# dhmodi/spark-timeseries

Hardware: AMD Instinct MI355X
Metric: series fitted/sec, ARIMA(2,1,2) CSS-CGD, 1M x 1024 pts (higher is better)
Workload: dtype f64; 1 GPU; ARIMA(2,1,2)+c css-cgd, 1048576 series x 1024 pts per GPU (BASELINE.json configs[1]/[2]); series_per_gpu=1048576, series_total=1048576, series_len=1024, parallelism=series-sharded x1, no collective, breeze_overlap=smear, fit_kernel=k_cg_fit (LDS slots, 1 wave/SIMD), fit_pipeline=6, hw_queues=8, series_done=1048576

## Files before the change

spark-timeseries_amd/csrc/arima_device.hpp:

```cpp
#pragma once

#include <hip/hip_runtime.h>
#include <stdint.h>

#include <type_traits>

#include "../../include/sparkts_arima.h"
#include "arima_launch.hpp"
#include "cg_lane.hpp"

namespace sts {

constexpr int kChunk = 16;


__device__ __forceinline__ double dlog(double x) {
    const double ln2_hi = 6.93147180369123816490e-01, ln2_lo = 1.90821492927058770002e-10,
                 two54 = 1.80143985094819840000e+16, Lg1 = 6.666666666666735130e-01,
                 Lg2 = 3.999999999940941908e-01, Lg3 = 2.857142874366239149e-01,
                 Lg4 = 2.222219843214978396e-01, Lg5 = 1.818357216161805012e-01,
                 Lg6 = 1.531383769920937332e-01, Lg7 = 1.479819860511658591e-01;
    int64_t bits = __double_as_longlong(x);
    int32_t hx = (int32_t)(bits >> 32);
    uint32_t lx = (uint32_t)bits;
    int32_t k = 0;
    if (hx < 0x00100000) {
        if (((hx & 0x7fffffff) | lx) == 0) return -two54 / 0.0;
        if (hx < 0) return (x - x) / 0.0;
        k -= 54;
        x *= two54;
        hx = (int32_t)(__double_as_longlong(x) >> 32);
    }
    if (hx >= 0x7ff00000) return x + x;
    k += (hx >> 20) - 1023;
    hx &= 0x000fffff;
    int32_t i = (hx + 0x95f64) & 0x100000;
    {
        uint64_t u = (uint64_t)__double_as_longlong(x);
        u = ((uint64_t)(uint32_t)(hx | (i ^ 0x3ff00000)) << 32) | (u & 0xffffffffull);
        x = __longlong_as_double((long long)u);
    }
    k += (i >> 20);
    double f = x - 1.0;
    double dk;
    if ((0x000fffff & (2 + hx)) < 3) {
        if (f == 0.0) {
            if (k == 0) return 0.0;
            dk = (double)k;
            return dk * ln2_hi + dk * ln2_lo;
        }
        double R = f * f * (0.5 - 0.33333333333333333 * f);
        if (k == 0) return f - R;
        dk = (double)k;
        return dk * ln2_hi - ((R - dk * ln2_lo) - f);
    }
    double s = f / (2.0 + f);
    dk = (double)k;
    double z = s * s;
    i = hx - 0x6147a;
    double w = z * z;
    int32_t j = 0x6b851 - hx;
    double t1 = w * (Lg2 + w * (Lg4 + w * Lg6));
    double t2 = z * (Lg1 + w * (Lg3 + w * (Lg5 + w * Lg7)));
    i |= j;
    double R = t2 + t1;
    if (i > 0) {
        double hfsq = 0.5 * f * f;
        if (k == 0) return f - (hfsq - s * (hfsq + R));
        return dk * ln2_hi - ((hfsq - (s * (hfsq + R) + dk * ln2_lo)) - f);
    }
    if (k == 0) return f - s * (f - R);
    return dk * ln2_hi - ((s * (f - R) - dk * ln2_lo) - f);
}

__device__ __forceinline__ double css_to_loglik(double css, int n) {
    double sigma2 = css / (double)n;
    return (double)(-n / 2) * dlog(2.0 * 3.141592653589793 * sigma2) - css / (2.0 * sigma2);
}

struct Chunk {
    double v[kChunk];
};

__device__ __forceinline__ void load_chunk(const double *__restrict__ p, Chunk &out) {
    const double2 *q = reinterpret_cast<const double2 *>(p);
#pragma unroll
    for (int u = 0; u < kChunk / 2; ++u) {
        const double2 t = q[u];
        out.v[2 * u] = t.x;
        out.v[2 * u + 1] = t.y;
    }
}

template <int D, class Fn>
__device__ __forceinline__ void stream_elems(const double *__restrict__ row, int first, int last, Fn &&fn) {
    if (first >= last) return;
    const int c_first = first / kChunk;
    const int c_last = (last - 1) / kChunk;
    const int nch = c_last - c_first + 1;
    const double *base = row + c_first * kChunk;
    Chunk ring[D];
#pragma unroll
    for (int j = 0; j < D; ++j) load_chunk(base + (j < nch ? j : nch - 1) * kChunk, ring[j]);
    const int head = first - c_first * kChunk;
    const int tail = last - c_last * kChunk;
    for (int c0 = 0; c0 < nch; c0 += D) {
#pragma unroll
        for (int j = 0; j < D; ++j) {
            const int ch = c0 + j;
            if (ch < nch) {
                const bool full = (ch > 0 || head == 0) && (ch < nch - 1 || tail == kChunk);
                if (full) {
#pragma unroll
                    for (int u = 0; u < kChunk; ++u) fn(ring[j].v[u]);
                } else {
                    const int lo = (ch == 0) ? head : 0;
                    const int hi = (ch == nch - 1) ? tail : kChunk;
#pragma unroll
                    for (int u = 0; u < kChunk; ++u)
                        if (u >= lo && u < hi) fn(ring[j].v[u]);
                }
            }
            const int nx = ch + D;
            load_chunk(base + (nx < nch ? nx : nch - 1) * kChunk, ring[j]);
        }
    }
}

__device__ __forceinline__ double drow_at(const double *__restrict__ raw, int dd, int i) {
    return dd ? raw[i + 1] - raw[i] : raw[i];
}

template <int D, class Fn>
__device__ __forceinline__ void stream_row(const double *__restrict__ raw, int dd, int first, int last, Fn &&fn) {
    if (first >= last) return;
    const int off = (int)((reinterpret_cast<uintptr_t>(raw) >> 3) & (kChunk - 1));
    double prev = raw[first];
    stream_elems<D>(raw - off, first + dd + off, last + dd + off, [&](double x) {
        const double v = dd ? x - prev : x;
        prev = x;
        fn(v);
    });
}

constexpr int kPrefetchF = 3;
constexpr int kPrefetchG = 1;

template <int P, int Q, int I, bool G, bool SMEAR, bool RAW = false, int DPF = (G ? kPrefetchG : kPrefetchF)>
__device__ __forceinline__ void css_pass(const double *__restrict__ row, int n,
                                         const double (&c)[I + P + Q > 0 ? I + P + Q : 1], double &css_out,
                                         double (&g)[I + P + Q > 0 ? I + P + Q : 1], int dd = 0) {
    constexpr int K = I + P + Q;
    constexpr int KA = K > 0 ? K : 1;
    constexpr int M = (P > Q ? P : Q);
    constexpr int PA = P > 0 ? P : 1;
    double yl[PA];
#pragma unroll
    for (int j = 0; j < PA; ++j) {
        if constexpr (RAW) yl[j] = (j < P && M - 1 - j < n) ? drow_at(row, dd, M - 1 - j) : 0.0;
        else yl[j] = (j < P) ? row[M - 1 - j] : 0.0;
    }
    double e1 = 0.0, e2 = 0.0, css = 0.0, sigma2 = 0.0;
    const double yh0 = 0.0 + (double)I * c[0];
    const double nd = (double)n;
    constexpr int DER = G ? (SMEAR ? (Q > 0 ? 2 : 1) : Q + 1) : 1;
    double dE[DER][KA];
    if constexpr (G) {
#pragma unroll
        for (int r = 0; r < DER; ++r)
#pragma unroll
            for (int j = 0; j < KA; ++j) dE[r][j] = 0.0;
    }
#pragma unroll
    for (int j = 0; j < KA; ++j) g[j] = 0.0;

    auto step = [&](double yi) {
        if constexpr (!G) {
            double yh = yh0;
#pragma unroll
            for (int j = 0; j < P; ++j) yh = yh + yl[j] * c[I + j];
#pragma unroll
            for (int j = 0; j < Q; ++j) yh = yh + (j == 0 ? e1 : e2) * c[I + P + j];
            const double e = yi - yh;
            css = css + e * e;
            e2 = e1;
            e1 = e;
        } else {
#pragma unroll
            for (int j = 0; j < K; ++j)
#pragma unroll
                for (int kk = 0; kk < Q; ++kk) dE[0][j] = dE[0][j] - c[I + P + kk] * dE[SMEAR ? DER - 1 : kk + 1][j];
            double yh = yh0;
            if constexpr (K > 0) dE[0][0] = dE[0][0] - (double)I;
#pragma unroll
            for (int j = 0; j < P; ++j) {
                yh = yh + yl[j] * c[I + j];
                dE[0][I + j] = dE[0][I + j] - yl[j];
            }
#pragma unroll
            for (int j = 0; j < Q; ++j) {
                const double mj = (j == 0 ? e1 : e2);
                yh = yh + mj * c[I + P + j];
                dE[0][I + P + j] = dE[0][I + P + j] - mj;
            }
            const double e = yi - yh;
            const double e_sq = e * e;
            sigma2 = sigma2 + e_sq / nd;
            css = css + e_sq;
            e2 = e1;
            e1 = e;
#pragma unroll
            for (int j = 0; j < K; ++j) g[j] = g[j] + dE[0][j] * e;
            if constexpr (SMEAR) {
                if constexpr (Q > 0) {
#pragma unroll
                    for (int j = 0; j < KA; ++j) dE[1][j] = dE[0][j];
                }
            } else {
#pragma unroll
                for (int r = Q; r >= 1; --r)
#pragma unroll
                    for (int j = 0; j < KA; ++j) dE[r][j] = dE[r - 1][j];
            }
#pragma unroll
            for (int j = 0; j < KA; ++j) dE[0][j] = 0.0;
        }
        if constexpr (P > 0) {
#pragma unroll
            for (int j = PA - 1; j >= 1; --j) yl[j] = yl[j - 1];
            yl[0] = yi;
        }
    };
    if constexpr (RAW) stream_row<DPF>(row, dd, M, n, step);
    else stream_elems<DPF>(row, M, n, step);
    css_out = css;
    if constexpr (G) {
#pragma unroll
        for (int j = 0; j < KA; ++j) g[j] = g[j] / -sigma2;
    }
}

template <int P, int Q, int I, int NCH, int DPF = kPrefetchF>
__device__ __forceinline__ void css_pass_multi(const double *__restrict__ row, int n,
                                               const double (&c)[NCH][I + P + Q > 0 ? I + P + Q : 1],
                                               double (&css_out)[NCH], int dd = 0) {
    constexpr int M = (P > Q ? P : Q);
    constexpr int PA = P > 0 ? P : 1;
    double yl[PA];
#pragma unroll
    for (int j = 0; j < PA; ++j) yl[j] = (j < P && M - 1 - j < n) ? drow_at(row, dd, M - 1 - j) : 0.0;
    double e1[NCH], e2[NCH], css[NCH], yh0[NCH];
#pragma unroll
    for (int h = 0; h < NCH; ++h) {
        e1[h] = e2[h] = css[h] = 0.0;
        yh0[h] = 0.0 + (double)I * c[h][0];
    }
    auto step = [&](double yi) {
#pragma unroll
        for (int h = 0; h < NCH; ++h) {
            double yh = yh0[h];
#pragma unroll
            for (int j = 0; j < P; ++j) yh = yh + yl[j] * c[h][I + j];
#pragma unroll
            for (int j = 0; j < Q; ++j) yh = yh + (j == 0 ? e1[h] : e2[h]) * c[h][I + P + j];
            const double e = yi - yh;
            css[h] = css[h] + e * e;
            e2[h] = e1[h];
            e1[h] = e;
        }
        if constexpr (P > 0) {
#pragma unroll
            for (int j = PA - 1; j >= 1; --j) yl[j] = yl[j - 1];
            yl[0] = yi;
        }
    };
    stream_row<DPF>(row, dd, M, n, step);
#pragma unroll
    for (int h = 0; h < NCH; ++h) css_out[h] = css[h];
}

template <int P, int Q, int I>
__device__ __forceinline__ double css_row_lds(const double *row, int n,
                                              const double (&c)[I + P + Q > 0 ? I + P + Q : 1]) {
    constexpr int M = (P > Q ? P : Q);
    constexpr int PA = P > 0 ? P : 1;
    double yl[PA];
#pragma unroll
    for (int j = 0; j < PA; ++j) yl[j] = (j < P && M - 1 - j >= 0 && M - 1 - j < n) ? row[M - 1 - j] : 0.0;
    double e1 = 0.0, e2 = 0.0, css = 0.0;
    const double yh0 = 0.0 + (double)I * c[0];
// ... 264 lines not shown
    constexpr int DR = SMEAR ? 1 : (Q > 0 ? Q : 1);
    double yl[PA];
#pragma unroll
    for (int j = 0; j < PA; ++j) yl[j] = (j < P && M - 1 - j >= 0 && M - 1 - j < n) ? row[M - 1 - j] : 0.0;
    double e1 = 0.0, e2 = 0.0, css = 0.0, sigma2 = 0.0, g = 0.0;
    double dl[DR];
#pragma unroll
    for (int r = 0; r < DR; ++r) dl[r] = 0.0;
    const double yh0 = 0.0 + (double)I * c[0];
    const double nd = (double)n;
#pragma unroll 4
    for (int t = M; t < n; ++t) {
        const double yi = row[t];
        double d0 = 0.0;
#pragma unroll
        for (int kk = 0; kk < Q; ++kk) d0 = d0 - c[I + P + kk] * dl[SMEAR ? 0 : kk];
        double dv = 0.0;
        if constexpr (I) dv = (col == 0) ? 1.0 : dv;
        double yh = yh0;
#pragma unroll
        for (int j = 0; j < P; ++j) {
            yh = yh + yl[j] * c[I + j];
            dv = (col == I + j) ? yl[j] : dv;
        }
#pragma unroll
        for (int j = 0; j < Q; ++j) {
            const double mj = (j == 0 ? e1 : e2);
            yh = yh + mj * c[I + P + j];
            dv = (col == I + P + j) ? mj : dv;
        }
        d0 = d0 - dv;
        const double e = yi - yh;
        const double e_sq = e * e;
        sigma2 = sigma2 + e_sq / nd;
        css = css + e_sq;
        e2 = e1;
        e1 = e;
        g = g + d0 * e;
        if constexpr (Q > 0) {
            if constexpr (SMEAR) {
                dl[0] = d0;
            } else {
#pragma unroll
                for (int r = DR - 1; r >= 1; --r) dl[r] = dl[r - 1];
                dl[0] = d0;
            }
        }
        if constexpr (P > 0) {
#pragma unroll
            for (int j = PA - 1; j >= 1; --j) yl[j] = yl[j - 1];
            yl[0] = yi;
        }
    }
    css_out = css;
    g_out = g / -sigma2;
}

constexpr int kPrefetchHR = 2;

template <int C>
struct HouseholderState {
    double a[C];
    double vtop[C];
    double alpha[C][C];
    double dot[C];
};

template <int C>
__device__ __forceinline__ void hh_apply(const HouseholderState<C> &H, int s, double (&x)[C], double &y) {
#pragma unroll
    for (int j = 0; j < C; ++j) {
        if (j < s) {
            const double v = x[j];
#pragma unroll
            for (int c = j + 1; c < C; ++c) x[c] = x[c] - H.alpha[j][c] * v;
            y = y + H.dot[j] * v;
        }
    }
}

template <class Gen, class Fn>
__device__ __forceinline__ void gen_stream(const Gen &gen, const double *__restrict__ row, int first, int last,
                                           Fn &&fn) {
    if constexpr (Gen::kFuse) stream_row<kPrefetchHR>(row, gen.dd, first, last, fn);
    else stream_row<kPrefetchHR>(row, 0, first, last, fn);
}

template <int C, int S, class Gen>
__device__ __forceinline__ int ols_stage(Gen &gen, const double *__restrict__ row, int n, int R,
                                         HouseholderState<C> &H) {
    if constexpr (S == C) {
        return ARIMA_ST_OK;
    } else {
        double xs[C], ys;
        gen.row_at(S, xs, ys);
        hh_apply<C>(H, S, xs, ys);
        const double xss = xs[S];
        double xnorm = 0.0 + xss * xss;
        if constexpr (S == 0 && Gen::kOnesFirst) {
            xnorm = (double)R;
        } else if (S + 1 < R) {
            gen.begin(S + 1);
            gen_stream(gen, row, gen.first_elem(S + 1), n, [&](double v) {
                double x[C], y;
                gen.push(v, x, y);
                hh_apply<C>(H, S, x, y);
                xnorm = xnorm + x[S] * x[S];
            });
        }
        const double a = (xss > 0) ? -sqrt(xnorm) : sqrt(xnorm);
        H.a[S] = a;
        if (a == 0.0) return ARIMA_ST_SINGULAR;
        const double vt = xss - a;
        H.vtop[S] = vt;
        double al[C], dt;
#pragma unroll
        for (int c = 0; c < C; ++c) al[c] = (c > S) ? 0.0 - xs[c] * vt : 0.0;
        dt = 0.0 + ys * vt;
        if (S + 1 < R) {
            gen.begin(S + 1);
            gen_stream(gen, row, gen.first_elem(S + 1), n, [&](double v) {
                double x[C], y;
                gen.push(v, x, y);
                hh_apply<C>(H, S, x, y);
                const double vs = x[S];
#pragma unroll
                for (int c = S + 1; c < C; ++c) al[c] = al[c] - x[c] * vs;
                dt = dt + y * vs;
            });
        }
        const double den = a * vt;
#pragma unroll
        for (int c = 0; c < C; ++c) H.alpha[S][c] = (c > S) ? al[c] / den : 0.0;
        H.dot[S] = dt / den;
        return ols_stage<C, S + 1>(gen, row, n, R, H);
    }
}

template <int C, class Gen>
__device__ __forceinline__ int stream_ols(Gen &gen, const double *__restrict__ row, int n, int R, double (&beta)[C]) {
    HouseholderState<C> H;
    const int st = ols_stage<C, 0>(gen, row, n, R, H);
    if (st != ARIMA_ST_OK) return st;
    double rrow[C][C];
    double ytop[C];
#pragma unroll
    for (int i = 0; i < C; ++i) {
        double x[C], y;
        gen.row_at(i, x, y);
        hh_apply<C>(H, i, x, y);
#pragma unroll
        for (int c = i + 1; c < C; ++c) x[c] = x[c] - H.alpha[i][c] * H.vtop[i];
        y = y + H.dot[i] * H.vtop[i];
#pragma unroll
        for (int c = 0; c < C; ++c) rrow[i][c] = x[c];
        ytop[i] = y;
    }
#pragma unroll
    for (int r = C - 1; r >= 0; --r) {
        ytop[r] = ytop[r] / H.a[r];
        const double yRow = ytop[r];
        beta[r] = yRow;
#pragma unroll
        for (int i = 0; i < C; ++i)
            if (i < r) ytop[i] = ytop[i] - yRow * rrow[i][r];
    }
    return ARIMA_ST_OK;
}


template <int m, int INTERCEPT, bool F = true>
struct ARGen {
    static constexpr int C = INTERCEPT + m;
    static constexpr bool kOnesFirst = INTERCEPT != 0;
    static constexpr bool kFuse = F;
    const double *__restrict__ y;
    int dd = 0;
    double w[m + 1];
    __device__ __forceinline__ double at(int i) const {
        if constexpr (F) return drow_at(y, dd, i);
        else return y[i];
    }
    __device__ __forceinline__ void row_at(int r, double (&x)[C], double &yv) const {
        if constexpr (INTERCEPT) x[0] = 1.0;
#pragma unroll
        for (int l = 1; l <= m; ++l) x[INTERCEPT + l - 1] = at(r + m - l);
        yv = at(r + m);
    }
    __device__ __forceinline__ int first_elem(int r) const { return r + m; }
    __device__ __forceinline__ void begin(int r) {
#pragma unroll
        for (int l = 1; l <= m; ++l) w[l] = at(r + m - l);
    }
    __device__ __forceinline__ void push(double v, double (&x)[C], double &yv) {
        w[0] = v;
        if constexpr (INTERCEPT) x[0] = 1.0;
#pragma unroll
        for (int l = 1; l <= m; ++l) x[INTERCEPT + l - 1] = w[l];
        yv = w[0];
#pragma unroll
        for (int l = m; l >= 1; --l) w[l] = w[l - 1];
    }
};

template <int P, int Q, int I, bool F = true>
struct HRGen {
    static constexpr int M = (P > Q ? P : Q);
    static constexpr int m = M + 1;
    static constexpr int C = I + P + Q;
    static constexpr int QA = Q > 0 ? Q : 1;
    static constexpr bool kOnesFirst = I != 0;
    static constexpr bool kFuse = F;
    const double *__restrict__ y;
    int dd = 0;
    double a[m];
    double c;
    double w[m + 2];
    double ew[QA + 1];
    __device__ __forceinline__ double at(int i) const {
        if constexpr (F) return drow_at(y, dd, i);
        else return y[i];
    }
    __device__ __forceinline__ double err_at(int s) const {
        double acc = 0.0;
#pragma unroll
        for (int j = 0; j < m; ++j) acc = acc + at(s + m - 1 - j) * a[j];
        return at(s + m) - (acc + c);
    }
    __device__ __forceinline__ void row_at(int r, double (&x)[C > 0 ? C : 1], double &yv) const {
        if constexpr (I) x[0] = 1.0;
#pragma unroll
        for (int l = 1; l <= P; ++l) x[I + l - 1] = at(m + r + M - l);
#pragma unroll
        for (int l = 1; l <= Q; ++l) x[I + P + l - 1] = err_at(r + M - l);
        yv = at(m + r + M);
    }
    __device__ __forceinline__ int first_elem(int r) const { return m + M + r; }
    __device__ __forceinline__ void begin(int r) {
        const int e = m + M + r;
#pragma unroll
        for (int l = 1; l <= m + 1; ++l) w[l] = at(e - l);
#pragma unroll
        for (int l = 2; l <= Q; ++l) ew[l] = err_at(r + M - l);
    }
    __device__ __forceinline__ void push(double v, double (&x)[C > 0 ? C : 1], double &yv) {
        w[0] = v;
        if constexpr (Q > 0) {
            double acc = 0.0;
#pragma unroll
            for (int j = 0; j < m; ++j) acc = acc + w[2 + j] * a[j];
            ew[1] = w[1] - (acc + c);
        }
        if constexpr (I) x[0] = 1.0;
#pragma unroll
        for (int l = 1; l <= P; ++l) x[I + l - 1] = w[l];
#pragma unroll
        for (int l = 1; l <= Q; ++l) x[I + P + l - 1] = ew[l];
        yv = w[0];
#pragma unroll
        for (int l = m + 1; l >= 1; --l) w[l] = w[l - 1];
#pragma unroll
        for (int l = QA; l >= 2; --l) ew[l] = ew[l - 1];
    }
};

template <int N>
__device__ __forceinline__ bool roots_outside_unit_circle(const double (&poly)[N + 1]) {
    double a[N + 1];
#pragma unroll
    for (int i = 0; i <= N; ++i) {
        a[i] = poly[i];
        if (!finite(a[i])) return false;
    }
#pragma unroll
    for (int mm = N; mm >= 1; --mm) {
        const double kk = a[mm];
        if (!(fabs(kk) < 1.0)) return false;
        const double den = 1.0 - kk * kk;
        double b[N + 1];
#pragma unroll
        for (int i = 0; i <= N; ++i) b[i] = (i < mm) ? (a[i] - kk * a[mm - i]) / den : 0.0;
#pragma unroll
        for (int i = 0; i <= N; ++i) a[i] = b[i];
    }
    return true;
}

template <int P, int Q, int I>
__device__ __forceinline__ uint8_t model_flags(const double (&c)[I + P + Q > 0 ? I + P + Q : 1]) {
    uint8_t f = 0;
    bool st = true, inv = true;
    if constexpr (P > 0) {
        double poly[P + 1];
        poly[0] = 1.0;
#pragma unroll
        for (int j = 0; j < P; ++j) poly[1 + j] = -1.0 * c[I + j];
        st = roots_outside_unit_circle<P>(poly);
    }
    if constexpr (Q > 0) {
        double poly[Q + 1];
        poly[0] = 1.0;
#pragma unroll
        for (int j = 0; j < Q; ++j) poly[1 + j] = c[I + P + j];
        inv = roots_outside_unit_circle<Q>(poly);
    }
// ... 122 lines not shown
```

spark-timeseries_amd/csrc/arima_generic.hip:

```cpp
#include <algorithm>

#include "arima_device.hpp"
#include "arima_launch.hpp"

namespace sts {

namespace {
inline unsigned gen_grid(int64_t n, int block) { return (unsigned)((n + block - 1) / block); }
}

#define STS_GEN_CHECK()                                                                                    \
    do {                                                                                                   \
        if (hipGetLastError() != hipSuccess) return ARIMA_E_DEVICE;                                        \
    } while (0)

__device__ double gen_grad(const GRow &r, int n, int p, int q, int I, const double *c, int smear, double *g,
                           double *dE) {
    const int k = I + p + q, M = p > q ? p : q;
    const int rows = smear ? (q > 0 ? 2 : 1) : q + 1;
    for (int j = 0; j < rows * k; ++j) dE[j] = 0.0;
    for (int j = 0; j < k; ++j) g[j] = 0.0;
    double e1 = 0.0, e2 = 0.0, sigma2 = 0.0, css = 0.0;
    const double nd = (double)n;
    const double yh0 = 0.0 + (double)I * c[0];
    for (int t = M; t < n; ++t) {
        for (int j = 0; j < k; ++j)
            for (int kk = 0; kk < q; ++kk) dE[j] = dE[j] - c[I + p + kk] * dE[(smear ? 1 : kk + 1) * k + j];
        double yh = yh0;
        if (k > 0) dE[0] = dE[0] - (double)I;
        for (int j = 0; j < p; ++j) {
            const double v = r.at(t - 1 - j);
            yh = yh + v * c[I + j];
            dE[I + j] = dE[I + j] - v;
        }
        for (int j = 0; j < q; ++j) {
            const double mj = (j == 0 ? e1 : e2);
            yh = yh + mj * c[I + p + j];
            dE[I + p + j] = dE[I + p + j] - mj;
        }
        const double e = r.at(t) - yh;
        const double e_sq = e * e;
        sigma2 = sigma2 + e_sq / nd;
        css = css + e_sq;
        e2 = e1;
        e1 = e;
        for (int j = 0; j < k; ++j) g[j] = g[j] + dE[j] * e;
        if (smear) {
            if (q > 0)
                for (int j = 0; j < k; ++j) dE[k + j] = dE[j];
        } else {
            for (int rr = q; rr >= 1; --rr)
                for (int j = 0; j < k; ++j) dE[rr * k + j] = dE[(rr - 1) * k + j];
        }
        for (int j = 0; j < k; ++j) dE[j] = 0.0;
    }
    for (int j = 0; j < k; ++j) g[j] = g[j] / -sigma2;
    return css;
}

struct GenQR {
    double a[kGenMaxK], vtop[kGenMaxK], dot[kGenMaxK];
    double alpha[kGenMaxK * kGenMaxK];
};

__device__ __forceinline__ void gen_hh_apply(const GenQR &H, int C, int s, double *x, double &y) {
    for (int j = 0; j < s; ++j) {
        const double v = x[j];
        for (int c = j + 1; c < C; ++c) x[c] = x[c] - H.alpha[j * C + c] * v;
        y = y + H.dot[j] * v;
    }
}

template <class RowGen>
__device__ int gen_ols(const RowGen &gen, int R, int C, bool ones_first, GenQR &H, double *beta) {
    double x[kGenMaxK], xs[kGenMaxK], al[kGenMaxK];
    for (int S = 0; S < C; ++S) {
        double ys;
        gen.row(S, xs);
        ys = gen.resp(S);
        gen_hh_apply(H, C, S, xs, ys);
        const double xss = xs[S];
        double xnorm = 0.0 + xss * xss;
        if (S == 0 && ones_first) {
            xnorm = (double)R;
        } else {
            for (int r = S + 1; r < R; ++r) {
                double y = gen.resp(r);
                gen.row(r, x);
                gen_hh_apply(H, C, S, x, y);
                xnorm = xnorm + x[S] * x[S];
            }
        }
        const double a = (xss > 0) ? -sqrt(xnorm) : sqrt(xnorm);
        H.a[S] = a;
        if (a == 0.0) return ARIMA_ST_SINGULAR;
        const double vt = xss - a;
        H.vtop[S] = vt;
        for (int c = 0; c < C; ++c) al[c] = (c > S) ? 0.0 - xs[c] * vt : 0.0;
        double dt = 0.0 + ys * vt;
        for (int r = S + 1; r < R; ++r) {
            double y = gen.resp(r);
            gen.row(r, x);
            gen_hh_apply(H, C, S, x, y);
            const double vs = x[S];
            for (int c = S + 1; c < C; ++c) al[c] = al[c] - x[c] * vs;
            dt = dt + y * vs;
        }
        const double den = a * vt;
        for (int c = 0; c < C; ++c) H.alpha[S * C + c] = (c > S) ? al[c] / den : 0.0;
        H.dot[S] = dt / den;
    }
    double ytop[kGenMaxK];
    for (int i = C - 1; i >= 0; --i) {
        double y = gen.resp(i);
        gen.row(i, x);
        gen_hh_apply(H, C, i, x, y);
        for (int c = i + 1; c < C; ++c) x[c] = x[c] - H.alpha[i * C + c] * H.vtop[i];
        y = y + H.dot[i] * H.vtop[i];
        for (int c = 0; c < C; ++c) H.alpha[i * C + c] = x[c];
        ytop[i] = y;
    }
    for (int r = C - 1; r >= 0; --r) {
        ytop[r] = ytop[r] / H.a[r];
        const double yRow = ytop[r];
        beta[r] = yRow;
// ... 435 lines not shown
```

spark-timeseries_amd/csrc/arima_kernels_impl.hpp:

```cpp
#pragma once
#include <hip/hip_runtime.h>

#include <algorithm>
#include <utility>

#include "arima_device.hpp"
#include "arima_launch.hpp"
#include <type_traits>

namespace sts {

template <int V>
using IC = std::integral_constant<int, V>;

template <int P, int Q, int I, bool F>
__global__ __launch_bounds__(256) void k_hr_init(const double *__restrict__ y, int64_t ld, int n, int64_t N,
                                                 double *__restrict__ init_out, int32_t *__restrict__ status_out,
                                                 int dd, FitPrep prep) {
    constexpr int K = I + P + Q;
    constexpr int KA = K > 0 ? K : 1;
    constexpr int M = P > Q ? P : Q;
    constexpr int m = M + 1;
    fit_prep(prep);
    for (int64_t sid = (int64_t)blockIdx.x * blockDim.x + threadIdx.x; sid < N;
         sid += (int64_t)gridDim.x * blockDim.x) {
    const double *row = y + sid * ld;
    int st = hr_shape_status(n, P, Q, I);
    double beta[KA];
#pragma unroll
    for (int j = 0; j < KA; ++j) beta[j] = __builtin_nan("");
    if (st == ARIMA_ST_OK) {
        double ab[1 + m];
        ARGen<m, 1, F> genA;
        genA.y = row;
        genA.dd = F ? dd : 0;
        st = stream_ols<1 + m>(genA, row, n, n - m, ab);
        if (st == ARIMA_ST_OK) {
            HRGen<P, Q, I, F> genB;
            genB.y = row;
            genB.dd = F ? dd : 0;
            genB.c = ab[0];
#pragma unroll
            for (int j = 0; j < m; ++j) genB.a[j] = ab[1 + j];
            double bb[KA];
            if constexpr (K > 0) {
                st = stream_ols<K>(genB, row, n, n - m - M, bb);
                if (st == ARIMA_ST_OK) {
#pragma unroll
                    for (int j = 0; j < K; ++j) beta[j] = bb[j];
                }
            }
        }
    }
#pragma unroll
    for (int j = 0; j < K; ++j) init_out[sid * K + j] = beta[j];
    status_out[sid] = st;
    }
}

template <int P, int I>
__global__ __launch_bounds__(256) void k_ar_fit(const double *__restrict__ y, int64_t ld, int n, int64_t N,
                                                double *__restrict__ coef_out, double *__restrict__ ll_out,
                                                int32_t *__restrict__ status_out, int32_t *__restrict__ n_eval_out,
                                                int32_t *__restrict__ n_grad_out, uint8_t *__restrict__ flags_out,
                                                int dd) {
    constexpr int K = I + P;
    const int64_t sid = (int64_t)blockIdx.x * blockDim.x + threadIdx.x;
    if (sid >= N) return;
    const double *row = y + sid * ld;
    int st = ar_shape_status(n, P, I);
    double beta[K];
#pragma unroll
    for (int j = 0; j < K; ++j) beta[j] = __builtin_nan("");
    double ll = __builtin_nan("");
    uint8_t fl = 0;
    if (st == ARIMA_ST_OK) {
        double b[K];
        ARGen<P, I> gen;
        gen.y = row;
        gen.dd = dd;
        st = stream_ols<K>(gen, row, n, n - P, b);
        if (st == ARIMA_ST_OK) {
#pragma unroll
            for (int j = 0; j < K; ++j) beta[j] = b[j];
            double css, g[K];
            css_pass<P, 0, I, false, false, true>(row, n, beta, css, g, dd);
            ll = css_to_loglik(css, n);
            fl = model_flags<P, 0, I>(beta);
        }
    }
#pragma unroll
    for (int j = 0; j < K; ++j) coef_out[sid * K + j] = beta[j];
    ll_out[sid] = ll;
    status_out[sid] = st;
    if (n_eval_out) n_eval_out[sid] = 0;
    if (n_grad_out) n_grad_out[sid] = 0;
    if (flags_out) flags_out[sid] = fl;
}

template <int K>
__device__ __forceinline__ void write_fit(int64_t sid, int status, const double (&coef)[K], double ll, int n_eval,
                                          int n_grad, uint8_t flags, double *coef_out, double *ll_out,
                                          int32_t *status_out, int32_t *n_eval_out, int32_t *n_grad_out,
                                          uint8_t *flags_out, int path = 1) {
    const bool ok = status == ARIMA_ST_OK;
#pragma unroll
    for (int j = 0; j < K; ++j) coef_out[sid * K + j] = ok ? coef[j] : __builtin_nan("");
    ll_out[sid] = ok ? ll : __builtin_nan("");
    status_out[sid] = status;
    if (n_eval_out) n_eval_out[sid] = n_eval;
    if (n_grad_out) n_grad_out[sid] = n_grad;
    if (flags_out) flags_out[sid] = ok ? flags : 0;
#ifdef STS_TIMING
    ll_out[sid] = (double)__builtin_amdgcn_s_memrealtime();
    if (flags_out) flags_out[sid] = (uint8_t)path;
#endif
}

template <int K>
constexpr int spec_ns() { return 2; }
template <int K>
constexpr int spec_nc() { return 4; }

// ... 677 lines not shown
        const int nsel = base < 64 ? base : 64;
        __builtin_amdgcn_fence(__ATOMIC_RELEASE, "wavefront");
        __builtin_amdgcn_wave_barrier();
        __builtin_amdgcn_fence(__ATOMIC_ACQUIRE, "wavefront");
        const bool served = lane < nsel;
        const int my = served ? assign[wave][lane] : 0;
        FitSlotCore<K> &S = ws[my].c;
        const double *row = served ? y + S.sid * ld : y;
        double c[K], css, g[K];
        if (served) {
            S.s.request_point(c);
        } else {
#pragma unroll
            for (int j = 0; j < K; ++j) c[j] = 0.0;
        }
        double resp_f = 0.0;
#ifdef STS_TIMING
        const unsigned long long t_b = now();
        tm_sel += t_b - t_a;
#endif
        if (doG) {
            css_pass<P, Q, I, true, SMEAR, true>(row, n, c, css, g, dd);
            resp_f = css_to_loglik(css, n);
            wave_g += lane0;
            lane_g += served;
            rides += (served && S.s.req == REQ_F) ? 1ull : 0ull;
        } else {
            int nsp = served ? (int)S.s.rq_nspec : 0;
            nsp = nsp < nchc - 1 ? nsp : nchc - 1;
            int nch = 1;
#pragma unroll
            for (int h = 1; h <= NS; ++h)
                if (__ballot(nsp >= h) != 0ull) nch = h + 1;
            auto multi = [&](auto NCHc) {
                constexpr int NCH = decltype(NCHc)::value;
                double cm[NCH][K], cssm[NCH];
#pragma unroll
                for (int j = 0; j < K; ++j) cm[0][j] = c[j];
#pragma unroll
                for (int h = 1; h < NCH; ++h) {
                    if (h <= nsp) {
                        double cs[K];
                        S.s.spec_point(h - 1, cs);
#pragma unroll
                        for (int j = 0; j < K; ++j) cm[h][j] = cs[j];
                    } else {
#pragma unroll
                        for (int j = 0; j < K; ++j) cm[h][j] = c[j];
                    }
                }
                css_pass_multi<P, Q, I, NCH>(row, n, cm, cssm, dd);
                css = cssm[0];
                if (served) {
#pragma unroll
                    for (int h = 1; h < NCH; ++h)
                        if (h <= nsp) S.s.spec_store(h - 1, css_to_loglik(cssm[h], n));
                }
            };
            if constexpr (NS >= 2) {
                if (nch == 3) multi(IC<3>{});
                else if (nch == 2) multi(IC<2>{});
                else multi(IC<1>{});
            } else if constexpr (NS == 1) {
                if (nch == 2) multi(IC<2>{});
                else multi(IC<1>{});
            } else {
                multi(IC<1>{});
            }
            resp_f = css_to_loglik(css, n);
            if (nch > 1) wave_m += lane0; else wave_f += lane0;
            lane_f += served;
            chains += served ? (unsigned long long)(1 + nsp) : 0ull;
            wave_chains += lane0 ? (unsigned long long)(64 * nch) : 0ull;
        }
        low_passes += (lane0 && nsel < 32) ? 1ull : 0ull;
#ifdef STS_TIMING
        const unsigned long long t_c = now();
        if (doG) tm_g += t_c - t_b; else tm_f += t_c - t_b;
#endif
        bool need = false;
        if (served) {
            CGLane<K, NS, spec_nc<K>()> &L = S.s;
            L.req = REQ_NONE;
            L.advance(resp_f, g);
            if (L.done()) {
                double pt[K];
#pragma unroll
                for (int j = 0; j < K; ++j) pt[j] = L.point[j];
                write_fit<K>(S.sid, L.status, pt, L.prev_obj, L.n_eval, L.n_grad,
                             L.status == ARIMA_ST_OK ? model_flags<P, Q, I>(pt) : (uint8_t)0, coef_out, ll_out,
                             status_out, n_eval_out, n_grad_out, flags_out);
                timing_stamp<K>(S, coef_out);
                evals += L.n_eval;
                grads += L.n_grad;
                hits += L.spec_hits;
                done++;
                need = true;
            }
        }
#ifdef STS_TIMING
        const unsigned long long t_s = now();
        tm_step += t_s - t_c;
#endif
        refill(my, need);
#ifdef STS_TIMING
        tm_refill += now() - t_s;
#endif
        if (has_express) {
            unsigned long long wants = 0, filled = 0, fault = 0;
            if (lane0) {
                wants = ld_agent(&ctl[20]);
                filled = ld_agent(&ctl[21]);
                fault = ld_agent(&ctl[26]);
            }
            wants = __shfl(wants, 0);
            filled = __shfl(filled, 0);
            fault = __shfl(fault, 0);
            if (wants > filled && filled < xring && fault == 0) {
                const int donate_min = __any(drained) ? don_drained : don_evals;
                unsigned long long key = 0;
#pragma unroll
                for (int j = 0; j < NJ; ++j) {
                    const int slot = lane + 64 * j;
                    if (slot < SPW && ws[slot].c.sid >= 0 && ws[slot].c.s.req != REQ_NONE &&
                        ws[slot].c.s.n_eval >= donate_min) {
                        const unsigned long long kk = ((unsigned long long)ws[slot].c.s.n_eval << 16) | (unsigned)(slot + 1);
                        key = kk > key ? kk : key;
                    }
                }
#pragma unroll
                for (int off = 32; off >= 1; off >>= 1) {
                    const unsigned long long o = __shfl_xor(key, off);
                    key = o > key ? o : key;
                }
                unsigned long long jx = 0;
                int claimed = 0;
                if (lane0 && key) {
                    unsigned long long f = filled;
                    while (f < wants && f < xring) {
                        const unsigned long long prev = cas_agent(&ctl[21], f, f + 1ull);
                        if (prev == f) {
                            jx = f;
                            claimed = 1;
                            break;
                        }
                        f = prev;
                        wants = ld_agent(&ctl[20]);
                    }
                }
                claimed = __shfl(claimed, 0);
                jx = __shfl(jx, 0);
                if (claimed) {
                    const int bs = (int)(key & 0xffffull) - 1;
                    const unsigned e = (unsigned)(jx % xring);
#ifdef STS_TIMING
                    if (lane == (bs & 63)) ws[bs].c.t_donate = (double)__builtin_amdgcn_s_memrealtime();
                    wave_sync_lds();
#endif
                    publish_core<K>(reinterpret_cast<unsigned long long *>(xq + (size_t)e * kExpressEntryBytes), &ws[bs].c,
                                    lane, jx + 1);
                    asm volatile("s_waitcnt vmcnt(0)" ::: "memory");
                    if (lane0) st_agent(&xready[e], (unsigned)(jx + 1));
                    if (lane == (bs & 63)) {
                        ws[bs].c.sid = -1;
                        ws[bs].c.s.req = REQ_NONE;
                    }
                    wave_sync_lds();
// ... 70 lines not shown
}

template <int P, int Q, int I, bool SMEAR>
__global__ __launch_bounds__(256) void k_css_grad(const double *__restrict__ y, int64_t ld, int n, int64_t N,
                                                  const double *__restrict__ coef, double *__restrict__ g_out) {
    constexpr int K = I + P + Q;
    constexpr int KA = K > 0 ? K : 1;
    const int64_t sid = (int64_t)blockIdx.x * blockDim.x + threadIdx.x;
    if (sid >= N) return;
    double c[KA], g[KA], css;
#pragma unroll
    for (int j = 0; j < KA; ++j) c[j] = (j < K) ? coef[sid * K + j] : 0.0;
    css_pass<P, Q, I, true, SMEAR>(y + sid * ld, n, c, css, g);
#pragma unroll
    for (int j = 0; j < K; ++j) g_out[sid * K + j] = g[j];
}

template <int P, int Q, int I>
__global__ __launch_bounds__(256) void k_model_flags(const double *__restrict__ coef, int64_t N,
                                                     uint8_t *__restrict__ flags_out) {
    constexpr int K = I + P + Q;
    constexpr int KA = K > 0 ? K : 1;
    const int64_t sid = (int64_t)blockIdx.x * blockDim.x + threadIdx.x;
    if (sid >= N) return;
    double c[KA];
#pragma unroll
    for (int j = 0; j < KA; ++j) c[j] = (j < K) ? coef[sid * K + j] : 0.0;
    flags_out[sid] = model_flags<P, Q, I>(c);
}


#ifdef STS_DEV
template <class Fn>
int with_order(int v, Fn &&fn) {
    return v == STS_DEV_Q ? fn(IC<STS_DEV_Q>{}) : ARIMA_E_UNSUPPORTED;
}
template <class Fn>
int with_smear(int v, Fn &&fn) {
    return v ? fn(IC<1>{}) : ARIMA_E_UNSUPPORTED;
}
#else
template <class Fn>
int with_order(int v, Fn &&fn) {
    switch (v) {
    case 0: return fn(IC<0>{});
    case 1: return fn(IC<1>{});
    case 2: return fn(IC<2>{});
    case 3: return fn(IC<3>{});
    case 4: return fn(IC<4>{});
    case 5: return fn(IC<5>{});
    default: return ARIMA_E_UNSUPPORTED;
    }
}
#endif
template <class Fn>
int with_bool(int v, Fn &&fn) {
    return v ? fn(IC<1>{}) : fn(IC<0>{});
}
#ifndef STS_DEV
template <class Fn>
int with_smear(int v, Fn &&fn) {
    return with_bool(v, fn);
}
#endif

inline unsigned grid_for(int64_t n, int block) { return (unsigned)((n + block - 1) / block); }

#define STS_CHECK_LAUNCH()                                                                                 \
    do {                                                                                                   \
        hipError_t e_ = hipGetLastError();                                                                 \
        if (e_ != hipSuccess) return ARIMA_E_DEVICE;                                                       \
    } while (0)

template <int P, bool F>
int launch_hr_init_PF(const double *y, int64_t ld, int n, int64_t N, int q, int I, double *init_out,
                      int32_t *status_out, hipStream_t s, int hr_grid, int dd, const FitPrep &prep) {
    return with_order(q, [&](auto Qc) {
        return with_bool(I, [&](auto Ic) {
            constexpr int Q = decltype(Qc)::value, II = decltype(Ic)::value;
            const int block = hr_grid > 0 ? 64 : 256;
            const unsigned grid =
                hr_grid > 0 ? std::min<unsigned>(grid_for(N, 64), (unsigned)hr_grid) : grid_for(N, 256);
            hipLaunchKernelGGL((k_hr_init<P, Q, II, F>), dim3(grid), dim3(block), 0, s, y, ld, n, N, init_out,
                               status_out, F ? dd : 0, prep);
            STS_CHECK_LAUNCH();
            return ARIMA_OK;
        });
    });
}

template <int P>
int launch_hr_init_P(const double *y, int64_t ld, int n, int64_t N, int q, int I, double *init_out,
                     int32_t *status_out, hipStream_t s, int hr_grid, int dd, const FitPrep &prep) {
    return dd ? launch_hr_init_PF<P, true>(y, ld, n, N, q, I, init_out, status_out, s, hr_grid, dd, prep)
              : launch_hr_init_PF<P, false>(y, ld, n, N, q, I, init_out, status_out, s, hr_grid, 0, prep);
}

template <int P>
int launch_ar_fit_P(const double *y, int64_t ld, int n, int64_t N, int I, double *coef_out, double *ll_out,
                    int32_t *status_out, int32_t *n_eval_out, int32_t *n_grad_out, uint8_t *flags_out,
                    hipStream_t s, int dd) {
    if constexpr (P == 0) {
        return ARIMA_E_INVALID_ARG;
    } else {
        return with_bool(I, [&](auto Ic) {
            constexpr int II = decltype(Ic)::value;
            hipLaunchKernelGGL((k_ar_fit<P, II>), dim3(grid_for(N, 256)), dim3(256), 0, s, y, ld, n, N, coef_out,
                               ll_out, status_out, n_eval_out, n_grad_out, flags_out, dd);
            STS_CHECK_LAUNCH();
            return ARIMA_OK;
        });
    }
}

template <int P, bool S>
int launch_cg_fit_PS(const double *y, int64_t ld, int n, int64_t N, int q, int I, const double *init,
                     const int32_t *init_status, double *coef_out, double *ll_out, int32_t *status_out,
                     int32_t *n_eval_out, int32_t *n_grad_out, uint8_t *flags_out, unsigned long long *ctl,
                     int grid_blocks, int express_blocks, unsigned char *xq, unsigned *xready, int join_express,
                     hipStream_t s, int dd) {
    return with_order(q, [&](auto Qc) {
        return with_bool(I, [&](auto Ic) {
            constexpr int Q = decltype(Qc)::value, II = decltype(Ic)::value;
            constexpr int K = P + Q + II;
            if constexpr (K == 0) {
                return ARIMA_E_INVALID_ARG;
            } else {
                constexpr int SPW = fit_slots_per_wave<K>();
                const int lds_per_wave = SPW * (int)sizeof(FitSlot<K>);
                if (n > express_max_n<K>(lds_per_wave)) express_blocks = 0;
                hipLaunchKernelGGL((k_cg_fit<P, Q, II, S, SPW>), dim3(grid_blocks + express_blocks),
                                   dim3(64 * kFitWaves), 0, s, y, ld, n, N, init, init_status, coef_out, ll_out,
                                   status_out, n_eval_out, n_grad_out, flags_out, ctl, xq, xready, grid_blocks,
                                   join_express, dd);
                STS_CHECK_LAUNCH();
                return ARIMA_OK;
            }
        });
    });
}

template <int P>
int launch_cg_fit_P(const double *y, int64_t ld, int n, int64_t N, int q, int I, int smear, const double *init,
                    const int32_t *init_status, double *coef_out, double *ll_out, int32_t *status_out,
                    int32_t *n_eval_out, int32_t *n_grad_out, uint8_t *flags_out, unsigned long long *ctl,
                    int grid_blocks, int express_blocks, unsigned char *xq, unsigned *xready, int join_express,
                    hipStream_t s, int dd) {
    return with_smear(smear, [&](auto Sc) {
        return launch_cg_fit_PS<P, (decltype(Sc)::value != 0)>(y, ld, n, N, q, I, init, init_status, coef_out, ll_out,
                                                               status_out, n_eval_out, n_grad_out, flags_out, ctl,
                                                               grid_blocks, express_blocks, xq, xready, join_express,
                                                               s, dd);
    });
}

template <int P>
int cg_fit_series_per_block_P(int q, int I) {
    return with_order(q, [&](auto Qc) {
        return with_bool(I, [&](auto Ic) {
            constexpr int Q = decltype(Qc)::value, II = decltype(Ic)::value;
            if constexpr (P + Q + II == 0) return 0;
            else return kFitWaves * fit_slots_per_wave<P + Q + II>();
        });
    });
}

template <int P>
// ... 74 lines not shown
```

Baseline: 10.98 million series fitted/sec.

## Replace per-step division by n with reciprocal FMA refinement; specialize differencing at compile time

The per-residual sigma2 accumulation divided e_sq by n each step, and on AMD GPUs an f64 divide expands to a long Newton/div_scale/div_fixup sequence. It now multiplies by a precomputed reciprocal refined with two FMA correction steps, and falls back to a true divide when a wave sees values outside a safe exponent range. The HR init generators and stream_row now take the differencing order as a template parameter, removing runtime dd branches, and CGLane::advance is forced inline at its call site. The FMA-refined quotient is meant to be exact but adds a wave-wide vote per step, and the extra inlining may raise register pressure in the one-wave-per-SIMD fit kernel.

```diff
diff --git a/spark-timeseries_amd/csrc/arima_device.hpp b/spark-timeseries_amd/csrc/arima_device.hpp
--- a/spark-timeseries_amd/csrc/arima_device.hpp
+++ b/spark-timeseries_amd/csrc/arima_device.hpp
@@ -8,6 +8,7 @@
 #include "../../include/sparkts_arima.h"
 #include "arima_launch.hpp"
 #include "cg_lane.hpp"
+#include "exact_divn.hpp"
 
 namespace sts {
 
@@ -131,16 +132,29 @@
     return dd ? raw[i + 1] - raw[i] : raw[i];
 }
 
+constexpr int kRuntimeDD = -1;
+
+template <int D, int DD, class Fn>
+__device__ __forceinline__ void stream_row(const double *__restrict__ raw, int first, int last, Fn &&fn) {
+    static_assert(DD == 0 || DD == 1, "fused differencing is first order");
+    if (first >= last) return;
+    const int off = (int)((reinterpret_cast<uintptr_t>(raw) >> 3) & (kChunk - 1));
+    if constexpr (DD == 0) {
+        stream_elems<D>(raw - off, first + off, last + off, fn);
+    } else {
+        double prev = raw[first];
+        stream_elems<D>(raw - off, first + 1 + off, last + 1 + off, [&](double x) {
+            const double v = x - prev;
+            prev = x;
+            fn(v);
+        });
+    }
+}
+
 template <int D, class Fn>
 __device__ __forceinline__ void stream_row(const double *__restrict__ raw, int dd, int first, int last, Fn &&fn) {
-    if (first >= last) return;
-    const int off = (int)((reinterpret_cast<uintptr_t>(raw) >> 3) & (kChunk - 1));
-    double prev = raw[first];
-    stream_elems<D>(raw - off, first + dd + off, last + dd + off, [&](double x) {
-        const double v = dd ? x - prev : x;
-        prev = x;
-        fn(v);
-    });
+    if (dd) stream_row<D, 1>(raw, first, last, fn);
+    else stream_row<D, 0>(raw, first, last, fn);
 }
 
 constexpr int kPrefetchF = 3;
@@ -162,7 +176,7 @@
     }
     double e1 = 0.0, e2 = 0.0, css = 0.0, sigma2 = 0.0;
     const double yh0 = 0.0 + (double)I * c[0];
-    const double nd = (double)n;
+    const DivN div_n((double)n);
     constexpr int DER = G ? (SMEAR ? (Q > 0 ? 2 : 1) : Q + 1) : 1;
     double dE[DER][KA];
     if constexpr (G) {
@@ -205,7 +219,7 @@
             }
             const double e = yi - yh;
             const double e_sq = e * e;
-            sigma2 = sigma2 + e_sq / nd;
+            sigma2 = sigma2 + div_n(e_sq);
             css = css + e_sq;
             e2 = e1;
             e1 = e;
@@ -636,8 +650,8 @@
 template <class Gen, class Fn>
 __device__ __forceinline__ void gen_stream(const Gen &gen, const double *__restrict__ row, int first, int last,
                                            Fn &&fn) {
-    if constexpr (Gen::kFuse) stream_row<kPrefetchHR>(row, gen.dd, first, last, fn);
-    else stream_row<kPrefetchHR>(row, 0, first, last, fn);
+    if constexpr (Gen::kDD == kRuntimeDD) stream_row<kPrefetchHR>(row, gen.dd, first, last, fn);
+    else stream_row<kPrefetchHR, Gen::kDD>(row, first, last, fn);
 }
 
 template <int C, int S, class Gen>
@@ -723,18 +737,15 @@
 }
 
 
-template <int m, int INTERCEPT, bool F = true>
+template <int m, int INTERCEPT, int DD = kRuntimeDD>
 struct ARGen {
     static constexpr int C = INTERCEPT + m;
     static constexpr bool kOnesFirst = INTERCEPT != 0;
-    static constexpr bool kFuse = F;
+    static constexpr int kDD = DD;
     const double *__restrict__ y;
     int dd = 0;
     double w[m + 1];
-    __device__ __forceinline__ double at(int i) const {
-        if constexpr (F) return drow_at(y, dd, i);
-        else return y[i];
-    }
+    __device__ __forceinline__ double at(int i) const { return drow_at(y, DD == kRuntimeDD ? dd : DD, i); }
     __device__ __forceinline__ void row_at(int r, double (&x)[C], double &yv) const {
         if constexpr (INTERCEPT) x[0] = 1.0;
 #pragma unroll
@@ -757,24 +768,21 @@
     }
 };
 
-template <int P, int Q, int I, bool F = true>
+template <int P, int Q, int I, int DD = kRuntimeDD>
 struct HRGen {
     static constexpr int M = (P > Q ? P : Q);
     static constexpr int m = M + 1;
     static constexpr int C = I + P + Q;
     static constexpr int QA = Q > 0 ? Q : 1;
     static constexpr bool kOnesFirst = I != 0;
-    static constexpr bool kFuse = F;
+    static constexpr int kDD = DD;
     const double *__restrict__ y;
     int dd = 0;
     double a[m];
     double c;
     double w[m + 2];
     double ew[QA + 1];
-    __device__ __forceinline__ double at(int i) const {
-        if constexpr (F) return drow_at(y, dd, i);
-        else return y[i];
-    }
+    __device__ __forceinline__ double at(int i) const { return drow_at(y, DD == kRuntimeDD ? dd : DD, i); }
     __device__ __forceinline__ double err_at(int s) const {
         double acc = 0.0;
 #pragma unroll
diff --git a/spark-timeseries_amd/csrc/arima_generic.hip b/spark-timeseries_amd/csrc/arima_generic.hip
--- a/spark-timeseries_amd/csrc/arima_generic.hip
+++ b/spark-timeseries_amd/csrc/arima_generic.hip
@@ -21,7 +21,7 @@
     for (int j = 0; j < rows * k; ++j) dE[j] = 0.0;
     for (int j = 0; j < k; ++j) g[j] = 0.0;
     double e1 = 0.0, e2 = 0.0, sigma2 = 0.0, css = 0.0;
-    const double nd = (double)n;
+    const DivN div_n((double)n);
     const double yh0 = 0.0 + (double)I * c[0];
     for (int t = M; t < n; ++t) {
         for (int j = 0; j < k; ++j)
@@ -40,7 +40,7 @@
         }
         const double e = r.at(t) - yh;
         const double e_sq = e * e;
-        sigma2 = sigma2 + e_sq / nd;
+        sigma2 = sigma2 + div_n(e_sq);
         css = css + e_sq;
         e2 = e1;
         e1 = e;
diff --git a/spark-timeseries_amd/csrc/arima_kernels_impl.hpp b/spark-timeseries_amd/csrc/arima_kernels_impl.hpp
--- a/spark-timeseries_amd/csrc/arima_kernels_impl.hpp
+++ b/spark-timeseries_amd/csrc/arima_kernels_impl.hpp
@@ -16,11 +16,12 @@
 template <int P, int Q, int I, bool F>
 __global__ __launch_bounds__(256) void k_hr_init(const double *__restrict__ y, int64_t ld, int n, int64_t N,
                                                  double *__restrict__ init_out, int32_t *__restrict__ status_out,
-                                                 int dd, FitPrep prep) {
+                                                 FitPrep prep) {
     constexpr int K = I + P + Q;
     constexpr int KA = K > 0 ? K : 1;
     constexpr int M = P > Q ? P : Q;
     constexpr int m = M + 1;
+    constexpr int DD = F ? 1 : 0;
     fit_prep(prep);
     for (int64_t sid = (int64_t)blockIdx.x * blockDim.x + threadIdx.x; sid < N;
          sid += (int64_t)gridDim.x * blockDim.x) {
@@ -31,14 +32,12 @@
     for (int j = 0; j < KA; ++j) beta[j] = __builtin_nan("");
     if (st == ARIMA_ST_OK) {
         double ab[1 + m];
-        ARGen<m, 1, F> genA;
+        ARGen<m, 1, DD> genA;
         genA.y = row;
-        genA.dd = F ? dd : 0;
         st = stream_ols<1 + m>(genA, row, n, n - m, ab);
         if (st == ARIMA_ST_OK) {
-            HRGen<P, Q, I, F> genB;
+            HRGen<P, Q, I, DD> genB;
             genB.y = row;
-            genB.dd = F ? dd : 0;
             genB.c = ab[0];
 #pragma unroll
             for (int j = 0; j < m; ++j) genB.a[j] = ab[1 + j];
@@ -882,7 +881,7 @@
         if (served) {
             CGLane<K, NS, spec_nc<K>()> &L = S.s;
             L.req = REQ_NONE;
-            L.advance(resp_f, g);
+            [[clang::always_inline]] L.advance(resp_f, g);
             if (L.done()) {
                 double pt[K];
 #pragma unroll
@@ -1119,7 +1118,7 @@
             const unsigned grid =
                 hr_grid > 0 ? std::min<unsigned>(grid_for(N, 64), (unsigned)hr_grid) : grid_for(N, 256);
             hipLaunchKernelGGL((k_hr_init<P, Q, II, F>), dim3(grid), dim3(block), 0, s, y, ld, n, N, init_out,
-                               status_out, F ? dd : 0, prep);
+                               status_out, prep);
             STS_CHECK_LAUNCH();
             return ARIMA_OK;
         });
diff --git a/spark-timeseries_amd/csrc/exact_divn.hpp b/spark-timeseries_amd/csrc/exact_divn.hpp
--- /dev/null
+++ b/spark-timeseries_amd/csrc/exact_divn.hpp
@@ -0,0 +1,37 @@
+#pragma once
+
+#include "cg_lane.hpp"
+
+namespace sts {
+
+struct DivN {
+    static constexpr double kSafeLo = 0x1p-960;
+    static constexpr double kSafeHi = 0x1p+1000;
+    double n, r;
+
+    STS_HD STS_FI explicit DivN(double nn) : n(nn), r(1.0 / nn) {}
+
+    STS_HD STS_FI static bool safe(double x) {
+        const double ax = dabs(x);
+        return ax >= kSafeLo && ax <= kSafeHi;
+    }
+
+    STS_HD STS_FI double fast(double x) const {
+        const double q0 = x * r;
+        const double q1 = __builtin_fma(__builtin_fma(-n, q0, x), r, q0);
+        return __builtin_fma(__builtin_fma(-n, q1, x), r, q1);
+    }
+
+    STS_HD STS_FI double operator()(double x) const {
+        double q = fast(x);
+        const bool ok = safe(x);
+#if defined(__HIP_DEVICE_COMPILE__)
+        if (__builtin_expect(__any(!ok), 0)) q = ok ? q : x / n;
+#else
+        if (!ok) q = x / n;
+#endif
+        return q;
+    }
+};
+
+}
```

Result: no change. 11.15 million series fitted/sec, median of 6 (+1.6%).
